# Scalsol/mega.pytorch

Hardware: AMD Instinct MI355X
Metric: frames/sec MEGA R-101 inference, 1000x600 VID clip (higher is better)
Workload: dtype bf16

## Files before the change

### mega/pytorch_amd/csrc/relation.hip

```cpp
#include <type_traits>

#include "launch.h"

namespace {

__device__ __forceinline__ void sincos_reduced(float a, float* sn, float* cs) {
  const float INV2PI = 0.15915494309189535f;
  const float TWO_PI_HI = 6.28318548202514648f;
  const float TWO_PI_LO = -1.7484555e-7f;
  const float n = rintf(a * INV2PI);
  float r = fmaf(-n, TWO_PI_HI, a);
  r = fmaf(-n, TWO_PI_LO, r);
  const float rev = r * INV2PI;
  *sn = __builtin_amdgcn_sinf(rev);
  *cs = __builtin_amdgcn_cosf(rev);
}

template <bool PRECISE>
__global__ __launch_bounds__(256) void pos_logits_kernel(const float4* __restrict__ rois_q,
                                                         const float4* __restrict__ rois_k,
                                                         const float* __restrict__ wgt, const float* __restrict__ bg,
                                                         const float* __restrict__ dim_mat, float* __restrict__ out,
                                                         int Nq, int Nk, int ldp) {
  __shared__ __attribute__((aligned(16))) float sw[64 * 16];
  __shared__ float sdim[8];
  for (int e = threadIdx.x; e < 1024; e += 256) sw[e] = wgt[e];
  if (threadIdx.x < 8) sdim[threadIdx.x] = dim_mat[threadIdx.x];
  __syncthreads();
  const int q = blockIdx.y;
  const int k = blockIdx.x * 256 + threadIdx.x;
  if (k >= Nk) return;
  const float4 bq = rois_q[q];
  const float4 bk = rois_k[k];
  const float wq = bq.z - bq.x + 1.f, hq = bq.w - bq.y + 1.f;
  const float cxq = 0.5f * (bq.x + bq.z), cyq = 0.5f * (bq.y + bq.w);
  const float wk = bk.z - bk.x + 1.f, hk = bk.w - bk.y + 1.f;
  const float cxk = 0.5f * (bk.x + bk.z), cyk = 0.5f * (bk.y + bk.w);
  float pm[4];
  pm[0] = logf(fabsf((cxq - cxk) / wq) + 1e-3f);
  pm[1] = logf(fabsf((cyq - cyk) / hq) + 1e-3f);
  pm[2] = logf(wq / wk);
  pm[3] = logf(hq / hk);
  float acc[16];
#pragma unroll
  for (int h = 0; h < 16; ++h) acc[h] = bg[h];
#pragma unroll
  for (int d = 0; d < 4; ++d) {
    const float pv = pm[d] * 100.0f;
#pragma unroll 2
    for (int i = 0; i < 8; ++i) {
      const float a = pv / sdim[i];
      float sn, cs;
      if (PRECISE) sincosf(a, &sn, &cs);
      else sincos_reduced(a, &sn, &cs);
      const float4* ws = reinterpret_cast<const float4*>(sw + (d * 16 + i) * 16);
      const float4* wc = reinterpret_cast<const float4*>(sw + (d * 16 + 8 + i) * 16);
#pragma unroll
      for (int h4 = 0; h4 < 4; ++h4) {
        const float4 a4 = ws[h4], c4 = wc[h4];
        acc[4 * h4 + 0] = fmaf(sn, a4.x, acc[4 * h4 + 0]);
        acc[4 * h4 + 1] = fmaf(sn, a4.y, acc[4 * h4 + 1]);
        acc[4 * h4 + 2] = fmaf(sn, a4.z, acc[4 * h4 + 2]);
        acc[4 * h4 + 3] = fmaf(sn, a4.w, acc[4 * h4 + 3]);
        acc[4 * h4 + 0] = fmaf(cs, c4.x, acc[4 * h4 + 0]);
        acc[4 * h4 + 1] = fmaf(cs, c4.y, acc[4 * h4 + 1]);
        acc[4 * h4 + 2] = fmaf(cs, c4.z, acc[4 * h4 + 2]);
        acc[4 * h4 + 3] = fmaf(cs, c4.w, acc[4 * h4 + 3]);
      }
    }
  }
#pragma unroll
  for (int h = 0; h < 16; ++h)
    out[((size_t)h * Nq + q) * ldp + k] = logf(fmaxf(acc[h], 0.f) + 1e-6f);
}

__device__ __forceinline__ float sin_shifted(float a, float shift_rev) {
  const float INV2PI = 0.15915494309189535f;
  const float TWO_PI_HI = 6.28318548202514648f;
  const float TWO_PI_LO = -1.7484555e-7f;
  const float n = rintf(a * INV2PI);
  float r = fmaf(-n, TWO_PI_HI, a);
  r = fmaf(-n, TWO_PI_LO, r);
  return __builtin_amdgcn_sinf(fmaf(r, INV2PI, shift_rev));
}

__device__ __forceinline__ float sin_rev(float x_rev) {
  return __builtin_amdgcn_sinf(__builtin_amdgcn_fractf(x_rev));
}

__device__ __forceinline__ float fast_log(float x) { return __builtin_amdgcn_logf(x) * 0.6931471805599453f; }
__device__ __forceinline__ float fast_div(float a, float b) { return a * __builtin_amdgcn_rcpf(b); }

typedef float f32x4_t __attribute__((ext_vector_type(4)));

__global__ __launch_bounds__(256) void pos_logits_mfma_kernel(const float4* __restrict__ rois_q,
                                                              const float4* __restrict__ rois_k,
                                                              const float* __restrict__ wgt,
                                                              const float* __restrict__ bg,
                                                              const float* __restrict__ dim_mat,
                                                              float* __restrict__ out, int Nq, int Nk, int ldp) {
  const int lane = threadIdx.x & 63, wave = threadIdx.x >> 6;
  const int row = lane & 15, g = lane >> 4;
  const int q = blockIdx.y;
  bf16x8_t bw[2];
#pragma unroll
  for (int s = 0; s < 2; ++s)
#pragma unroll
    for (int e = 0; e < 8; ++e) bw[s][e] = (__bf16)wgt[(32 * s + 8 * g + e) * 16 + row];
  float crev[8];
#pragma unroll
  for (int i = 0; i < 8; ++i) crev[i] = (100.0f * 0.15915494309189535f) / dim_mat[i];
  const float bias = bg[row];
  const float4 bq = rois_q[q];
  const float wq = bq.z - bq.x + 1.f, hq = bq.w - bq.y + 1.f;
  const float cxq = 0.5f * (bq.x + bq.z), cyq = 0.5f * (bq.y + bq.w);
  const float shift = (g & 1) ? 0.25f : 0.f;
#pragma unroll 1
  for (int t = 0; t < 4; ++t) {
    const int k0 = blockIdx.x * 256 + wave * 64 + t * 16;
    if (k0 >= Nk) break;
    const int k = min(k0 + row, Nk - 1);
    const float4 bk = rois_k[k];
    const float wk = bk.z - bk.x + 1.f, hk = bk.w - bk.y + 1.f;
    const float cxk = 0.5f * (bk.x + bk.z), cyk = 0.5f * (bk.y + bk.w);
    float pm[2];
    if (g >> 1) {
      pm[0] = fast_log(fabsf(fast_div(cyq - cyk, hq)) + 1e-3f);
      pm[1] = fast_log(fast_div(hq, hk));
    } else {
      pm[0] = fast_log(fabsf(fast_div(cxq - cxk, wq)) + 1e-3f);
      pm[1] = fast_log(fast_div(wq, wk));
    }
    f32x4_t acc = {bias, bias, bias, bias};
#pragma unroll
    for (int s = 0; s < 2; ++s) {
      bf16x8_t a;
#pragma unroll
      for (int i = 0; i < 8; ++i) a[i] = (__bf16)sin_rev(fmaf(pm[s], crev[i], shift));
      acc = __builtin_amdgcn_mfma_f32_16x16x32_bf16(a, bw[s], acc, 0, 0, 0);
    }
    float4 o;
    o.x = fast_log(fmaxf(acc[0], 0.f) + 1e-6f); o.y = fast_log(fmaxf(acc[1], 0.f) + 1e-6f);
    o.z = fast_log(fmaxf(acc[2], 0.f) + 1e-6f); o.w = fast_log(fmaxf(acc[3], 0.f) + 1e-6f);
    float* dst = out + ((size_t)row * Nq + q) * ldp + k0 + 4 * g;
    if (k0 + 4 * g + 3 < ldp) *reinterpret_cast<float4*>(dst) = o;
  }
}

template <typename HT> struct PosMma;
template <> struct PosMma<bf16_t> {
  typedef bf16x8_t vec;
  typedef __bf16 elem;
  __device__ static __forceinline__ f32x4_t run(const vec& a, const vec& b, const f32x4_t& c) { return __builtin_amdgcn_mfma_f32_16x16x32_bf16(a, b, c, 0, 0, 0); }
};
template <> struct PosMma<f16_t> {
  typedef f16x8_t vec;
  typedef _Float16 elem;
  __device__ static __forceinline__ f32x4_t run(const vec& a, const vec& b, const f32x4_t& c) { return __builtin_amdgcn_mfma_f32_16x16x32_f16(a, b, c, 0, 0, 0); }
};

template <typename HT>
__device__ __forceinline__ void pos_logits_tiled_body(const float4* __restrict__ rois_q,
                                                      const float4* __restrict__ rois_k,
                                                      const float* __restrict__ wgt, const float* __restrict__ bg,
                                                      const float* __restrict__ dim_mat, unsigned short* __restrict__ out_t,
                                                      int Nq, int Nk) {
  typedef typename PosMma<HT>::vec hvec;
  typedef typename PosMma<HT>::elem helem;
  __shared__ __attribute__((aligned(16))) unsigned short stage[16 * 2 * 8 * 32];
  const int lane = threadIdx.x & 63, wave = threadIdx.x >> 6;
  const int row = lane & 15, g = lane >> 4;
  const int q0 = blockIdx.y * 8, k00 = blockIdx.x * 64;
  hvec bw[2];
#pragma unroll
  for (int s = 0; s < 2; ++s)
#pragma unroll
    for (int e = 0; e < 8; ++e) bw[s][e] = (helem)wgt[(32 * s + 8 * g + e) * 16 + row];
  float crev[8];
#pragma unroll
  for (int i = 0; i < 8; ++i) crev[i] = (100.0f * 0.15915494309189535f) / dim_mat[i];
  const float bias = bg[row];
  const float shift = (g & 1) ? 0.25f : 0.f;
  float4 bqs[2], bks[4];
#pragma unroll
  for (int j = 0; j < 2; ++j) bqs[j] = rois_q[min(q0 + 2 * wave + j, Nq - 1)];
#pragma unroll
  for (int j = 0; j < 4; ++j) bks[j] = rois_k[min(k00 + j * 16 + row, Nk - 1)];
#pragma unroll
  for (int tile = 0; tile < 8; ++tile) {
    const int ql = 2 * wave + (tile >> 2);
    const int kb = (tile & 3) * 16;
    const float4 bq = bqs[tile >> 2];
    const float4 bk = bks[tile & 3];
    const float wq = bq.z - bq.x + 1.f, hq = bq.w - bq.y + 1.f;
    const float cxq = 0.5f * (bq.x + bq.z), cyq = 0.5f * (bq.y + bq.w);
    const float wk = bk.z - bk.x + 1.f, hk = bk.w - bk.y + 1.f;
    const float cxk = 0.5f * (bk.x + bk.z), cyk = 0.5f * (bk.y + bk.w);
    float pm[2];
    if (g >> 1) {
      pm[0] = fast_log(fabsf(fast_div(cyq - cyk, hq)) + 1e-3f);
      pm[1] = fast_log(fast_div(hq, hk));
    } else {
      pm[0] = fast_log(fabsf(fast_div(cxq - cxk, wq)) + 1e-3f);
      pm[1] = fast_log(fast_div(wq, wk));
    }
    f32x4_t acc = {bias, bias, bias, bias};
#pragma unroll
    for (int s = 0; s < 2; ++s) {
      hvec a;
#pragma unroll
      for (int i = 0; i < 8; ++i) a[i] = (helem)sin_rev(fmaf(pm[s], crev[i], shift));
      acc = PosMma<HT>::run(a, bw[s], acc);
    }
    const int kf = kb + 4 * g, ktl = kf >> 5, kk = kf & 31;
    uint2 pk;
    pk.x = Half16<HT>::pack2(fast_log(fmaxf(acc[0], 0.f) + 1e-6f), fast_log(fmaxf(acc[1], 0.f) + 1e-6f));
    pk.y = Half16<HT>::pack2(fast_log(fmaxf(acc[2], 0.f) + 1e-6f), fast_log(fmaxf(acc[3], 0.f) + 1e-6f));
    *reinterpret_cast<uint2*>(&stage[((row * 2 + ktl) * 8 + ql) * 32 + ((kk >> 2) & 1) * 16 + (kk >> 3) * 4]) = pk;
  }
  __syncthreads();
  const int ktiles = (Nk + 31) >> 5, kt0 = k00 >> 5;
  for (int idx = threadIdx.x; idx < 16 * 2 * 8 * 4; idx += 256) {
    const int chunk = idx & 3, ql = (idx >> 2) & 7, ktl = (idx >> 5) & 1, head = idx >> 6;
    if (q0 + ql < Nq && kt0 + ktl < ktiles)
      *reinterpret_cast<uint4*>(out_t + (((size_t)head * ktiles + kt0 + ktl) * Nq + q0 + ql) * 32 + chunk * 8) =
          *reinterpret_cast<const uint4*>(&stage[((head * 2 + ktl) * 8 + ql) * 32 + chunk * 8]);
  }
}

constexpr int POS_MAXB = 20;
struct PosBatch {
  struct { const float4* rq; const float4* rk; unsigned short* out; int Nq, Nk; } p[POS_MAXB];
};
template <typename HT>
__global__ __launch_bounds__(256) void pos_logits_tiled_batched_kernel(PosBatch b, const float* __restrict__ wgt,
                                                                       const float* __restrict__ bg,
                                                                       const float* __restrict__ dim_mat) {
  const auto& q = b.p[blockIdx.z];
  if ((int)blockIdx.x * 64 >= q.Nk || (int)blockIdx.y * 8 >= q.Nq) return;
  pos_logits_tiled_body<HT>(q.rq, q.rk, wgt, bg, dim_mat, q.out, q.Nq, q.Nk);
}

template <typename T> struct AttnCfg;
template <> struct AttnCfg<bf16_t> {
  static constexpr int KROW = 144;
  static constexpr int VROW = 72;
  static constexpr int NQF = 4;
  static constexpr int NPV = 2;
  static constexpr int NLD = 1;
};
template <> struct AttnCfg<f16_t> : AttnCfg<bf16_t> {};
template <> struct AttnCfg<float> {
  static constexpr int KROW = 272;
  static constexpr int VROW = 144;
  static constexpr int NQF = 8;
  static constexpr int NPV = 4;
  static constexpr int NLD = 2;
};

template <typename T> struct Mma32;
template <> struct Mma32<bf16_t> {
  __device__ static __forceinline__ void run(f32x16_t& acc, const uint4& a, const uint4& b) {
    acc = __builtin_amdgcn_mfma_f32_32x32x16_bf16(__builtin_bit_cast(bf16x8_t, a), __builtin_bit_cast(bf16x8_t, b), acc,
                                                  0, 0, 0);
  }
};
template <> struct Mma32<f16_t> {
  __device__ static __forceinline__ void run(f32x16_t& acc, const uint4& a, const uint4& b) {
    acc = __builtin_amdgcn_mfma_f32_32x32x16_f16(__builtin_bit_cast(f16x8_t, a), __builtin_bit_cast(f16x8_t, b), acc, 0, 0, 0);
  }
};
template <typename T> struct PairSum;
template <> struct PairSum<bf16_t> {
  __device__ static __forceinline__ float run(unsigned pk, float acc) {
    typedef __bf16 bf16x2_v __attribute__((ext_vector_type(2)));
    return __builtin_amdgcn_fdot2_f32_bf16(__builtin_bit_cast(bf16x2_v, pk), __builtin_bit_cast(bf16x2_v, 0x3f803f80u), acc, false);
  }
};
template <> struct PairSum<f16_t> {
  __device__ static __forceinline__ float run(unsigned pk, float acc) {
    return __builtin_amdgcn_fdot2(__builtin_bit_cast(f16x2_t, pk), __builtin_bit_cast(f16x2_t, 0x3c003c00u), acc, false);
  }
};
template <> struct PairSum<float> {
  __device__ static __forceinline__ float run(unsigned, float acc) { return acc; }
};
template <> struct Mma32<float> {
  __device__ static __forceinline__ void run(f32x16_t& acc, const uint4& a, const uint4& b) {
    acc = __builtin_amdgcn_mfma_f32_32x32x2f32(__uint_as_float(a.x), __uint_as_float(b.x), acc, 0, 0, 0);
    acc = __builtin_amdgcn_mfma_f32_32x32x2f32(__uint_as_float(a.y), __uint_as_float(b.y), acc, 0, 0, 0);
    acc = __builtin_amdgcn_mfma_f32_32x32x2f32(__uint_as_float(a.z), __uint_as_float(b.z), acc, 0, 0, 0);
    acc = __builtin_amdgcn_mfma_f32_32x32x2f32(__uint_as_float(a.w), __uint_as_float(b.w), acc, 0, 0, 0);
  }
};


struct AttnParams {
  const void* Q;
  const void* K;
  const void* Vt;
  const void* K2;
  const void* Vt2;
  const float* pos;
  const unsigned short* pos_t;
  const void* resid;
  const float* bias_v;
  void* out;
  float* part_o;
  float* part_ml;
  int ldq, ldk, ldv, ldv2, ldp, ldr, ldo;
  int Nq, Nk, N1, G;
  float scale;
  int nsplit, tiles_per_split;
  int io_f32;
};

template <typename T, bool POS_TILED, bool SEG>
__device__ __forceinline__ void attn_body(const AttnParams& p, const int split) {
  using C = AttnCfg<T>;
  constexpr int VE = 16 / (int)sizeof(T);
  constexpr int KV_PER_ROW = 64 * (int)sizeof(T) / 16;
  constexpr int VV_PER_ROW = 32 * (int)sizeof(T) / 16;
  constexpr int NLD = C::NLD;
  __shared__ __attribute__((aligned(16))) unsigned char Ks[2][32 * C::KROW];
  __shared__ __attribute__((aligned(16))) unsigned char Vs[2][64 * C::VROW];
  __shared__ __attribute__((aligned(16))) float sRow[4][32];

  const int tid = threadIdx.x, lane = tid & 63, wave = tid >> 6;
  const int h2 = lane >> 5, l31 = lane & 31;
  const int head = blockIdx.y;
  const int qw0 = blockIdx.x * 128 + wave * 32;
  const bool live = !POS_TILED || __builtin_amdgcn_readfirstlane(qw0) < p.Nq;
  const T* __restrict__ Qp = (const T*)p.Q;
  const int N1 = SEG ? p.N1 : p.Nk;
  const __amdgpu_buffer_rsrc_t rs_k = __builtin_amdgcn_make_buffer_rsrc(
      const_cast<void*>(p.K), 0, (int)((unsigned)N1 * (unsigned)p.ldk * (unsigned)sizeof(T)), 0x00020000);
  const __amdgpu_buffer_rsrc_t rs_v = __builtin_amdgcn_make_buffer_rsrc(
      const_cast<void*>(p.Vt), 0, (int)((unsigned)(p.G * 64) * (unsigned)p.ldv * (unsigned)sizeof(T)), 0x00020000);
  const __amdgpu_buffer_rsrc_t rs_k2 = __builtin_amdgcn_make_buffer_rsrc(
      const_cast<void*>(p.K2), 0, (int)((unsigned)(p.Nk - N1) * (unsigned)p.ldk * (unsigned)sizeof(T)), 0x00020000);
  const __amdgpu_buffer_rsrc_t rs_v2 = __builtin_amdgcn_make_buffer_rsrc(
      const_cast<void*>(p.Vt2), 0, (int)((unsigned)(p.G * 64) * (unsigned)p.ldv2 * (unsigned)sizeof(T)), 0x00020000);

  const int q_ld = min(qw0 + l31, p.Nq - 1);
  uint4 qf[C::NQF];
  {
    const unsigned char* qrow = (const unsigned char*)(Qp + (size_t)q_ld * p.ldq + head * 64);
#pragma unroll
    for (int v = 0; v < C::NQF; ++v) qf[v] = *reinterpret_cast<const uint4*>(qrow + v * 32 + h2 * 16);
  }

  auto load_tiles = [&](int k0, uint4 (&kreg)[NLD], uint4 (&vreg)[NLD]) {
    const bool in1 = !SEG || k0 + 32 <= N1, in2 = SEG && k0 >= N1;
#pragma unroll
    for (int i = 0; i < NLD; ++i) {
      const int idx = tid + 256 * i;
      {
        const int row = idx / KV_PER_ROW, vec = idx - row * KV_PER_ROW;
        const int key = k0 + row;
        const unsigned col = (unsigned)(head * 64 + vec * VE);
        const unsigned off1 = ((unsigned)key * (unsigned)p.ldk + col) * (unsigned)sizeof(T);
        const unsigned off2 = ((unsigned)(key - N1) * (unsigned)p.ldk + col) * (unsigned)sizeof(T);
        u32x4_t v;
        if (in1) {
          v = __builtin_amdgcn_raw_buffer_load_b128(rs_k, key < N1 ? off1 : 0xFFFFFFFFu, 0, 0);
        } else if (!SEG) {
          v = u32x4_t{0, 0, 0, 0};
        } else if (in2) {
          v = __builtin_amdgcn_raw_buffer_load_b128(rs_k2, key < p.Nk ? off2 : 0xFFFFFFFFu, 0, 0);
        } else {
          const u32x4_t a = __builtin_amdgcn_raw_buffer_load_b128(rs_k, key < N1 ? off1 : 0xFFFFFFFFu, 0, 0);
          const u32x4_t b = __builtin_amdgcn_raw_buffer_load_b128(rs_k2, key >= N1 && key < p.Nk ? off2 : 0xFFFFFFFFu, 0, 0);
          v = a | b;
        }
        kreg[i] = make_uint4(v.x, v.y, v.z, v.w);
      }
      {
        const int row = idx / VV_PER_ROW, vec = idx - row * VV_PER_ROW;
        const int key = k0 + vec * VE;
        const unsigned off1 = ((unsigned)(head * 64 + row) * (unsigned)p.ldv + (unsigned)key) * (unsigned)sizeof(T);
        const unsigned off2 = ((unsigned)(head * 64 + row) * (unsigned)p.ldv2 + (unsigned)(key - N1)) * (unsigned)sizeof(T);
        u32x4_t r;
        if (in1) {
          r = __builtin_amdgcn_raw_buffer_load_b128(rs_v, key < N1 ? off1 : 0xFFFFFFFFu, 0, 0);
        } else if (!SEG) {
          r = u32x4_t{0, 0, 0, 0};
        } else if (in2) {
          r = __builtin_amdgcn_raw_buffer_load_b128(rs_v2, key < p.Nk ? off2 : 0xFFFFFFFFu, 0, 0);
        } else {
          const u32x4_t a = __builtin_amdgcn_raw_buffer_load_b128(rs_v, key + VE <= N1 ? off1 : 0xFFFFFFFFu, 0, 0);
          const u32x4_t b = __builtin_amdgcn_raw_buffer_load_b128(rs_v2, key >= N1 && key < p.Nk ? off2 : 0xFFFFFFFFu, 0, 0);
          r = a | b;
          if (key < N1 && key + VE > N1) {
            T e[VE];
#pragma unroll
            for (int t = 0; t < VE; ++t) {
              const int kk = key + t;
              const T* src = kk < N1 ? (const T*)p.Vt + (size_t)(head * 64 + row) * p.ldv + kk
                                     : (const T*)p.Vt2 + (size_t)(head * 64 + row) * p.ldv2 + (kk - N1);
              e[t] = kk < p.Nk ? *src : (T)0;
            }
            r = *reinterpret_cast<const u32x4_t*>(e);
          }
        }
        uint4 v = make_uint4(r.x, r.y, r.z, r.w);
        if (k0 + 32 > p.Nk) {
          T* e = reinterpret_cast<T*>(&v);
#pragma unroll
          for (int t = 0; t < VE; ++t) e[t] = (key + t < p.Nk) ? e[t] : (T)0;
        }
        vreg[i] = v;
      }
    }
  };
  auto store_tiles = [&](int buf, const uint4 (&kreg)[NLD], const uint4 (&vreg)[NLD]) {
#pragma unroll
    for (int i = 0; i < NLD; ++i) {
      const int idx = tid + 256 * i;
      {
        const int row = idx / KV_PER_ROW, vec = idx - row * KV_PER_ROW;
        *reinterpret_cast<uint4*>(&Ks[buf][row * C::KROW + vec * 16]) = kreg[i];
      }
      {
        const int row = idx / VV_PER_ROW, vec = idx - row * VV_PER_ROW;
        unsigned char* dst = &Vs[buf][row * C::VROW + vec * 16];
        if (sizeof(T) == 2) {
          *reinterpret_cast<uint2*>(dst) = make_uint2(vreg[i].x, vreg[i].y);
          *reinterpret_cast<uint2*>(dst + 8) = make_uint2(vreg[i].z, vreg[i].w);
        } else {
          *reinterpret_cast<uint4*>(dst) = vreg[i];
        }
      }
    }
  };

  f32x16_t o0, o1;
#pragma unroll
  for (int r = 0; r < 16; ++r) { o0[r] = 0.f; o1[r] = 0.f; }
  float m_run = -INFINITY, l_run = 0.f;
  const float* pos_row = p.pos ? p.pos + ((size_t)head * p.Nq + q_ld) * p.ldp : nullptr;
  const int ktiles = (p.Nk + 31) >> 5;
  auto load_pos = [&](int kt, uint4 (&pr)[2]) {
    if (POS_TILED) {
      const int kc = min(kt, ktiles - 1);
      const uint4* src = reinterpret_cast<const uint4*>(p.pos_t + (((size_t)head * ktiles + kc) * p.Nq + q_ld) * 32 + h2 * 16);
      pr[0] = src[0];
      pr[1] = src[1];
    }
  };

  auto compute = [&](int cur, int k0, const uint4 (&pr)[2]) {
    f32x16_t st;
#pragma unroll
    for (int r = 0; r < 16; ++r) st[r] = 0.f;
    {
      const unsigned char* kb = &Ks[cur][l31 * C::KROW + h2 * 16];
#pragma unroll
      for (int v = 0; v < C::NQF; ++v) {
        const uint4 kf = *reinterpret_cast<const uint4*>(kb + v * 32);
        Mma32<T>::run(st, kf, qf[v]);
      }
    }
    float s[16];
#pragma unroll
    for (int rq = 0; rq < 4; ++rq) {
      float pe[4] = {0.f, 0.f, 0.f, 0.f};
      if (POS_TILED) {
        const unsigned short* pb = reinterpret_cast<const unsigned short*>(&pr[0]);
#pragma unroll
        for (int e = 0; e < 4; ++e) pe[e] = Half16<typename std::conditional<sizeof(T) == 2, T, bf16_t>::type>::one(pb[4 * rq + e]);
      } else if (pos_row) {
        const float4 pw = *reinterpret_cast<const float4*>(pos_row + k0 + 8 * rq + 4 * h2);
        pe[0] = pw.x; pe[1] = pw.y; pe[2] = pw.z; pe[3] = pw.w;
      }
#pragma unroll
      for (int e = 0; e < 4; ++e) s[4 * rq + e] = st[4 * rq + e] * p.scale + pe[e];
    }
    if (k0 + 32 > p.Nk) {
#pragma unroll
      for (int r = 0; r < 16; ++r) {
        const int key = k0 + 8 * (r >> 2) + 4 * h2 + (r & 3);
        s[r] = key < p.Nk ? s[r] : -INFINITY;
      }
    }
    float mt = s[0];
#pragma unroll
    for (int r = 1; r < 16; ++r) mt = fmaxf(mt, s[r]);
    mt = fmaxf(mt, __shfl_xor(mt, 32));
    const float m_new = fmaxf(m_run, mt);
    auto ex = [](float v) { return sizeof(T) == 2 ? __expf(v) : expf(v); };
    const float alpha = ex(m_run - m_new);
    float psum = 0.f;
    unsigned pk[8];
    if (sizeof(T) == 2) {
      const float kL2E = 1.44269504088896340736f, mneg = -m_new * kL2E;
#pragma unroll
      for (int r = 0; r < 16; ++r) s[r] = __builtin_amdgcn_exp2f(fmaf(s[r], kL2E, mneg));
    } else {
#pragma unroll
      for (int r = 0; r < 16; ++r) s[r] = ex(s[r] - m_new);
    }
    if (sizeof(T) == 2) {
#pragma unroll
      for (int d = 0; d < 8; ++d) {
        pk[d] = Half16<typename std::conditional<sizeof(T) == 2, T, bf16_t>::type>::pack2(s[2 * d], s[2 * d + 1]);
        psum = PairSum<T>::run(pk[d], psum);
      }
    } else {
#pragma unroll
      for (int r = 0; r < 16; ++r) psum += s[r];
    }
    l_run = l_run * alpha + psum;
    m_run = m_new;

    if (__builtin_amdgcn_ballot_w64(alpha != 1.f) != 0) {
      if (h2 == 0) sRow[wave][l31] = alpha;
      __builtin_amdgcn_wave_barrier();
#pragma unroll
      for (int rq = 0; rq < 4; ++rq) {
        const float4 a4 = *reinterpret_cast<const float4*>(&sRow[wave][8 * rq + 4 * h2]);
        o0[4 * rq + 0] *= a4.x; o0[4 * rq + 1] *= a4.y; o0[4 * rq + 2] *= a4.z; o0[4 * rq + 3] *= a4.w;
        o1[4 * rq + 0] *= a4.x; o1[4 * rq + 1] *= a4.y; o1[4 * rq + 2] *= a4.z; o1[4 * rq + 3] *= a4.w;
      }
      __builtin_amdgcn_wave_barrier();
    }

    const unsigned char* vb0 = &Vs[cur][l31 * C::VROW];
    const unsigned char* vb1 = &Vs[cur][(32 + l31) * C::VROW];
#pragma unroll
    for (int u = 0; u < C::NPV; ++u) {
      uint4 pa, v0, v1;
      if (sizeof(T) == 2) {
        pa.x = pk[4 * u + 0];
        pa.y = pk[4 * u + 1];
        pa.z = pk[4 * u + 2];
        pa.w = pk[4 * u + 3];
        const int off = (16 * u + 4 * h2) * 2;
        const uint2 a0 = *reinterpret_cast<const uint2*>(vb0 + off);
        const uint2 a1 = *reinterpret_cast<const uint2*>(vb0 + off + 16);
        const uint2 b0 = *reinterpret_cast<const uint2*>(vb1 + off);
        const uint2 b1 = *reinterpret_cast<const uint2*>(vb1 + off + 16);
        v0 = make_uint4(a0.x, a0.y, a1.x, a1.y);
        v1 = make_uint4(b0.x, b0.y, b1.x, b1.y);
      } else {
        pa.x = __float_as_uint(s[4 * u + 0]);
        pa.y = __float_as_uint(s[4 * u + 1]);
        pa.z = __float_as_uint(s[4 * u + 2]);
        pa.w = __float_as_uint(s[4 * u + 3]);
        const int off = (8 * u + 4 * h2) * 4;
        v0 = *reinterpret_cast<const uint4*>(vb0 + off);
        v1 = *reinterpret_cast<const uint4*>(vb1 + off);
      }
      Mma32<T>::run(o0, pa, v0);
      Mma32<T>::run(o1, pa, v1);
    }
  };

  const int ntiles = (p.Nk + 31) / 32;
  const int t0 = split * p.tiles_per_split;
  const int n = min(ntiles, t0 + p.tiles_per_split) - t0;
  uint4 ka[NLD], va[NLD], kb2[NLD], vb2[NLD];
  uint4 pA[2] = {}, pB[2] = {};
  load_tiles(t0 * 32, ka, va);
  load_pos(t0, pA);
  store_tiles(0, ka, va);
  load_tiles((t0 + 1) * 32, ka, va);
  load_pos(t0 + 1, pB);
  __syncthreads();
  for (int i = 0; i + 1 < n; i += 2) {
    load_tiles((t0 + i + 2) * 32, kb2, vb2);
    if (live) {
      compute(0, (t0 + i) * 32, pA);
      load_pos(t0 + i + 2, pA);
    }
    store_tiles(1, ka, va);
    __syncthreads();
    load_tiles((t0 + i + 3) * 32, ka, va);
    if (live) {
      compute(1, (t0 + i + 1) * 32, pB);
      load_pos(t0 + i + 3, pB);
    }
    store_tiles(0, kb2, vb2);
    __syncthreads();
  }
  if (!live) return;
  if (n & 1) compute(0, (t0 + n - 1) * 32, pA);

  const float l_tot = l_run + __shfl_xor(l_run, 32);
  if (p.nsplit > 1) {
    if (h2 == 0 && qw0 + l31 < p.Nq) {
      float* ml = p.part_ml + (size_t)split * 2 * p.G * p.Nq;
      ml[(size_t)head * p.Nq + qw0 + l31] = m_run;
      ml[(size_t)(p.G + head) * p.Nq + qw0 + l31] = l_tot;
    }
    float* po = p.part_o + (size_t)split * p.Nq * p.G * 64;
#pragma unroll
    for (int jj = 0; jj < 2; ++jj) {
      const int col = head * 64 + jj * 32 + l31;
#pragma unroll
      for (int r = 0; r < 16; ++r) {
        const int q = qw0 + (r & 3) + 8 * (r >> 2) + 4 * h2;
        if (q < p.Nq) po[(size_t)q * p.G * 64 + col] = (jj == 0 ? o0[r] : o1[r]);
      }
    }
    return;
  }
  if (h2 == 0) sRow[wave][l31] = 1.f / l_tot;
  __builtin_amdgcn_wave_barrier();
  const T* __restrict__ resid = (const T*)p.resid;
  T* __restrict__ out = (T*)p.out;
#pragma unroll
  for (int jj = 0; jj < 2; ++jj) {
    const int col = head * 64 + jj * 32 + l31;
    const float bv = p.bias_v ? p.bias_v[col] : 0.f;
#pragma unroll
    for (int r = 0; r < 16; ++r) {
      const int ql = (r & 3) + 8 * (r >> 2) + 4 * h2;
      const int q = qw0 + ql;
      if (q < p.Nq) {
        float v = (jj == 0 ? o0[r] : o1[r]) * sRow[wave][ql] + bv;
        if (p.io_f32) {
          if (resid) v += reinterpret_cast<const float*>(p.resid)[(size_t)q * p.ldr + col];
          reinterpret_cast<float*>(p.out)[(size_t)q * p.ldo + col] = v;
        } else {
          if (resid) v += Elem<T>::ld(resid + (size_t)q * p.ldr + col);
          Elem<T>::st(out + (size_t)q * p.ldo + col, v);
        }
      }
    }
  }
}

constexpr int ATTN_MAXB = 20;
constexpr int ATTN_MAXZ = 256;
struct AttnBatch {
  int n, nz;
  unsigned char zprob[ATTN_MAXZ], zsplit[ATTN_MAXZ];
  AttnParams p[ATTN_MAXB];
};
static_assert(sizeof(AttnBatch) <= 4096, "AttnBatch travels as the kernel argument");

template <typename T, bool POS_TILED, bool SEG>
__global__ __launch_bounds__(256, (POS_TILED && SEG) ? 3 : 2) void attn_batched_kernel(AttnBatch b) {
  const int z = blockIdx.z;
  const AttnParams& p = b.p[b.zprob[z]];
  if ((int)blockIdx.x * 128 >= p.Nq) return;
  attn_body<T, POS_TILED, SEG>(p, (int)b.zsplit[z]);
}

template <typename T>
__device__ __forceinline__ void attn_combine_body(const AttnParams& p) {
  const int D = p.G * 64;
  const size_t total = (size_t)p.Nq * D;
  for (size_t idx = (size_t)blockIdx.x * blockDim.x + threadIdx.x; idx < total; idx += (size_t)gridDim.x * blockDim.x) {
    const int q = (int)(idx / D), c = (int)(idx - (size_t)q * D), head = c >> 6;
    float M = -INFINITY;
    for (int s = 0; s < p.nsplit; ++s)
      M = fmaxf(M, p.part_ml[((size_t)s * 2 * p.G + head) * p.Nq + q]);
    float num = 0.f, den = 0.f;
    for (int s = 0; s < p.nsplit; ++s) {
      const float* ml = p.part_ml + (size_t)s * 2 * p.G * p.Nq;
      const float w = expf(ml[(size_t)head * p.Nq + q] - M);
      den += w * ml[(size_t)(p.G + head) * p.Nq + q];
      num += w * p.part_o[((size_t)s * p.Nq + q) * D + c];
    }
    float v = num / den + (p.bias_v ? p.bias_v[c] : 0.f);
    if (p.io_f32) {
      if (p.resid) v += reinterpret_cast<const float*>(p.resid)[(size_t)q * p.ldr + c];
      reinterpret_cast<float*>(p.out)[(size_t)q * p.ldo + c] = v;
    } else {
      if (p.resid) v += Elem<T>::ld((const T*)p.resid + (size_t)q * p.ldr + c);
      Elem<T>::st((T*)p.out + (size_t)q * p.ldo + c, v);
    }
  }
}

template <typename T>
__global__ __launch_bounds__(256) void attn_combine_batched_kernel(AttnBatch b) {
  const AttnParams& p = b.p[blockIdx.y];
  if (p.nsplit > 1) attn_combine_body<T>(p);
}

inline size_t align_up(size_t x, size_t a) { return (x + a - 1) / a * a; }

}

extern "C" int mega_position_logits(const float* rois_q, const float* rois_k, const float* wg_t, const float* bg,
                                    const float* dim_mat, float* out, int Nq, int Nk, int ldp, int precise,
                                    void* stream) {
  mega_clear_error();
  if (Nq == 0 || Nk == 0) return MEGA_OK;
  if (!rois_q || !rois_k || !wg_t || !bg || !dim_mat || !out || Nq < 0 || Nk < 0 || ldp < Nk) return MEGA_ERR_ARG;
  dim3 grid(cdiv(Nk, 256), Nq);
  if (precise)
    hipLaunchKernelGGL((pos_logits_kernel<true>), grid, dim3(256), 0, (hipStream_t)stream, (const float4*)rois_q,
                       (const float4*)rois_k, wg_t, bg, dim_mat, out, Nq, Nk, ldp);
  else if (ldp % 4 == 0 && (reinterpret_cast<size_t>(out) & 15) == 0)
    hipLaunchKernelGGL(pos_logits_mfma_kernel, grid, dim3(256), 0, (hipStream_t)stream, (const float4*)rois_q,
                       (const float4*)rois_k, wg_t, bg, dim_mat, out, Nq, Nk, ldp);
  else
    hipLaunchKernelGGL((pos_logits_kernel<false>), grid, dim3(256), 0, (hipStream_t)stream, (const float4*)rois_q,
                       (const float4*)rois_k, wg_t, bg, dim_mat, out, Nq, Nk, ldp);
  return mega_check_launch();
}

struct MegaPosDescC { const float* rois_q; const float* rois_k; void* out_bf16; int Nq, Nk; };

static int pos_tiled_launch(const MegaPosDescC* d, int n, const float* wg_t, const float* bg, const float* dim_mat,
                            int dtype, void* stream) {
  if (!d || n < 0 || n > POS_MAXB || !wg_t || !bg || !dim_mat) return MEGA_ERR_ARG;
  PosBatch b;
  int max_q = 0, max_k = 0;
  for (int i = 0; i < n; ++i) {
    if (!d[i].rois_q || !d[i].rois_k || !d[i].out_bf16 || d[i].Nq <= 0 || d[i].Nk <= 0 ||
        (reinterpret_cast<size_t>(d[i].out_bf16) & 15))
      return MEGA_ERR_ARG;
    b.p[i].rq = (const float4*)d[i].rois_q; b.p[i].rk = (const float4*)d[i].rois_k; b.p[i].out = (unsigned short*)d[i].out_bf16;
    b.p[i].Nq = d[i].Nq; b.p[i].Nk = d[i].Nk;
    max_q = d[i].Nq > max_q ? d[i].Nq : max_q;
    max_k = d[i].Nk > max_k ? d[i].Nk : max_k;
  }
  dim3 grid(cdiv(max_k, 64), cdiv(max_q, 8), n);
  return dispatch_half(dtype, [&](auto tag) {
    hipLaunchKernelGGL(pos_logits_tiled_batched_kernel<decltype(tag)>, grid, dim3(256), 0, (hipStream_t)stream, b, wg_t, bg,
                       dim_mat);
    return mega_check_launch();
  });
}

extern "C" int mega_position_logits_tiled_dt(const float* rois_q, const float* rois_k, const float* wg_t, const float* bg,
                                             const float* dim_mat, void* out16, int Nq, int Nk, int dtype, void* stream) {
  mega_clear_error();
  if (dtype != MEGA_BF16 && dtype != MEGA_F16) return MEGA_ERR_ARG;
  if (Nq == 0 || Nk == 0) return MEGA_OK;
  const MegaPosDescC d = {rois_q, rois_k, out16, Nq, Nk};
  return pos_tiled_launch(&d, 1, wg_t, bg, dim_mat, dtype, stream);
}

extern "C" int mega_position_logits_tiled_batched_dt(const void* descs, int n, const float* wg_t, const float* bg,
                                                     const float* dim_mat, int dtype, void* stream) {
  mega_clear_error();
  if (dtype != MEGA_BF16 && dtype != MEGA_F16) return MEGA_ERR_ARG;
  if (n == 0) return MEGA_OK;
  return pos_tiled_launch((const MegaPosDescC*)descs, n, wg_t, bg, dim_mat, dtype, stream);
}

constexpr int kAttnTargetBlocks = 48;

extern "C" int mega_relation_attention_splits(int Nq, int Nk, int groups) {
  if (Nq <= 0 || Nk <= 0 || groups <= 0) return 1;
  const int blocks = cdiv(Nq, 128) * groups;
  const int ntiles = cdiv(Nk, 32);
  int s = cdiv(kAttnTargetBlocks, blocks);
  if (s > ntiles / 4) s = ntiles / 4;
  if (s > 16) s = 16;
  return s < 1 ? 1 : s;
}

extern "C" size_t mega_relation_attention_workspace_bytes(int Nq, int Nk, int groups) {
  const int s = mega_relation_attention_splits(Nq, Nk, groups);
  if (s <= 1) return 0;
  return align_up((size_t)s * Nq * groups * 64 * sizeof(float), 256) +
         align_up((size_t)s * 2 * groups * Nq * sizeof(float), 256);
}

static int attn_fill(AttnParams& p, const void* q, int ldq, const void* k, int ldk, const void* vt, int ldv,
                     const float* pos, int ldp, const void* pos_tiled, const void* resid, int ldr, const float* bias_v,
                     void* out, int ldo, int Nq, int Nk, int groups, float scale, int dtype, void* ws, size_t ws_bytes,
                     int io_f32 = 0, int nk1 = 0, const void* k2 = nullptr, const void* vt2 = nullptr, int ldv2 = 0) {
  if (!q || !k || !vt || !out || Nq <= 0 || Nk <= 0 || groups <= 0) return MEGA_ERR_ARG;
  if (nk1 < 0 || nk1 > Nk) return MEGA_ERR_ARG;
  if (nk1 == 0 || nk1 == Nk) { nk1 = Nk; k2 = k; vt2 = vt; ldv2 = ldv; }
  else if (!k2 || !vt2 || ldv2 < Nk - nk1) return MEGA_ERR_ARG;
  p.N1 = nk1; p.K2 = k2; p.Vt2 = vt2; p.ldv2 = ldv2;
  p.io_f32 = (io_f32 != 0 && dtype != MEGA_F32) ? 1 : 0;
  const int ve = dtype != MEGA_F32 ? 8 : 4;
  if (ldq % ve || ldk % ve || ldv % ve || (pos && (ldp % 32 || ldp < Nk))) return MEGA_ERR_ARG;
  if (ldv < (nk1 == Nk ? ((Nk + ve - 1) / ve) * ve : nk1)) return MEGA_ERR_ARG;
  if (pos_tiled && (pos || dtype == MEGA_F32 || (reinterpret_cast<size_t>(pos_tiled) & 15))) return MEGA_ERR_ARG;
  p.pos_t = (const unsigned short*)pos_tiled;
  p.Q = q; p.ldq = ldq; p.K = k; p.ldk = ldk; p.Vt = vt; p.ldv = ldv; p.pos = pos; p.ldp = ldp;
  p.resid = resid; p.ldr = ldr; p.bias_v = bias_v; p.out = out; p.ldo = ldo; p.Nq = Nq; p.Nk = Nk; p.G = groups;
  p.scale = scale;
  const int want = mega_relation_attention_splits(Nq, Nk, groups);
  int nsplit = want;
  if (nsplit > 1 && (!ws || ws_bytes < mega_relation_attention_workspace_bytes(Nq, Nk, groups))) nsplit = 1;
  const int ntiles = cdiv(Nk, 32);
  p.tiles_per_split = cdiv(ntiles, nsplit);
  nsplit = cdiv(ntiles, p.tiles_per_split);
  p.nsplit = nsplit;
  p.part_o = (float*)ws;
  p.part_ml = nsplit > 1 ? (float*)((unsigned char*)ws + align_up((size_t)want * Nq * groups * 64 * sizeof(float), 256))
                         : nullptr;
  return MEGA_OK;
}

struct MegaAttnDescC {
  const void* q; const void* k; const void* vt; const float* pos; const void* pos_tiled; const void* resid;
  const float* bias_v; void* out; void* ws; size_t ws_bytes;
  int ldq, ldk, ldv, ldp, ldr, ldo, Nq, Nk;
  int io_f32, nk1;
  const void* k2; const void* vt2; int ldv2, reserved;
};

static int attn_launch(const MegaAttnDescC* d, int n, int groups, float scale, int dtype, void* stream) {
  if (!d || n < 0 || n > ATTN_MAXB) return MEGA_ERR_ARG;
  AttnBatch b;
  b.n = n;
  int nz = 0, max_q = 0, any_split = 0, any_seg = 0;
  size_t max_total = 0;
  const bool tiled = d[0].pos_tiled != nullptr;
  for (int i = 0; i < n; ++i) {
    if ((d[i].pos_tiled != nullptr) != tiled) return MEGA_ERR_ARG;
    const int rc = attn_fill(b.p[i], d[i].q, d[i].ldq, d[i].k, d[i].ldk, d[i].vt, d[i].ldv, d[i].pos, d[i].ldp,
                             d[i].pos_tiled, d[i].resid, d[i].ldr, d[i].bias_v, d[i].out, d[i].ldo, d[i].Nq, d[i].Nk,
                             groups, scale, dtype, d[i].ws, d[i].ws_bytes, d[i].io_f32, d[i].nk1, d[i].k2, d[i].vt2,
                             d[i].ldv2);
    if (rc != MEGA_OK) return rc;
    if (nz + b.p[i].nsplit > ATTN_MAXZ) return MEGA_ERR_ARG;
    for (int s2 = 0; s2 < b.p[i].nsplit; ++s2) { b.zprob[nz] = (unsigned char)i; b.zsplit[nz] = (unsigned char)s2; ++nz; }
    max_q = d[i].Nq > max_q ? d[i].Nq : max_q;
    any_split |= b.p[i].nsplit > 1;
    any_seg |= b.p[i].N1 != b.p[i].Nk;
    const size_t total = (size_t)d[i].Nq * groups * 64;
    max_total = total > max_total ? total : max_total;
  }
  b.nz = nz;
  hipStream_t st = (hipStream_t)stream;
  dim3 grid(cdiv(max_q, 128), groups, nz);
  return dispatch_elem(dtype, [&](auto tag) {
    using T = decltype(tag);
    auto kernel = any_seg ? attn_batched_kernel<T, false, true> : attn_batched_kernel<T, false, false>;
    if constexpr (!std::is_same<T, float>::value)
      if (tiled) kernel = any_seg ? attn_batched_kernel<T, true, true> : attn_batched_kernel<T, true, false>;
    hipLaunchKernelGGL(kernel, grid, dim3(256), 0, st, b);
    if (any_split)
      hipLaunchKernelGGL(attn_combine_batched_kernel<T>, dim3(grid1d(max_total, 4096), n), dim3(256), 0, st, b);
    return mega_check_launch();
  });
}

extern "C" int mega_relation_attention_batched(const void* descs, int n, int groups, float scale, int dtype,
                                               void* stream) {
  mega_clear_error();
  if (n == 0) return MEGA_OK;
  return attn_launch((const MegaAttnDescC*)descs, n, groups, scale, dtype, stream);
}

static int relation_attention_impl(const void* q, int ldq, const void* k, int ldk, const void* vt, int ldv,
                                   const float* pos, int ldp, const void* pos_tiled, const void* resid, int ldr,
                                   const float* bias_v, void* out, int ldo, int Nq, int Nk, int groups, float scale,
                                   int dtype, void* ws, size_t ws_bytes, void* stream) {
  mega_clear_error();
  if (Nq == 0) return MEGA_OK;
  MegaAttnDescC d = {};
  d.q = q; d.k = k; d.vt = vt; d.pos = pos; d.pos_tiled = pos_tiled; d.resid = resid; d.bias_v = bias_v; d.out = out;
  d.ws = ws; d.ws_bytes = ws_bytes;
  d.ldq = ldq; d.ldk = ldk; d.ldv = ldv; d.ldp = ldp; d.ldr = ldr; d.ldo = ldo; d.Nq = Nq; d.Nk = Nk;
  return attn_launch(&d, 1, groups, scale, dtype, stream);
}

extern "C" int mega_relation_attention(const void* q, int ldq, const void* k, int ldk, const void* vt, int ldv,
                                       const float* pos, int ldp, const void* resid, int ldr, const float* bias_v,
                                       void* out, int ldo, int Nq, int Nk, int groups, float scale, int dtype,
                                       void* ws, size_t ws_bytes, void* stream) {
  return relation_attention_impl(q, ldq, k, ldk, vt, ldv, pos, ldp, nullptr, resid, ldr, bias_v, out, ldo, Nq, Nk,
                                 groups, scale, dtype, ws, ws_bytes, stream);
}

extern "C" int mega_relation_attention_tiled_pos_dt(const void* q, int ldq, const void* k, int ldk, const void* vt,
                                                    int ldv, const void* pos_tiled16, const void* resid, int ldr,
                                                    const float* bias_v, void* out, int ldo, int Nq, int Nk, int groups,
                                                    float scale, int dtype, void* ws, size_t ws_bytes, void* stream) {
  if (dtype != MEGA_BF16 && dtype != MEGA_F16) return MEGA_ERR_ARG;
  return relation_attention_impl(q, ldq, k, ldk, vt, ldv, nullptr, 0, pos_tiled16, resid, ldr, bias_v, out, ldo, Nq,
                                 Nk, groups, scale, dtype, ws, ws_bytes, stream);
}
```

Baseline: 944.0.

## Prefetch tiled position logits via buffer-to-LDS DMA with counted waits

For the tiled positional-bias path, position logit tiles now go straight into per-wave LDS with buffer_load_lds, four tiles deep, instead of register loads two tiles ahead. Reads use counted vmcnt waits and inline-asm ds_reads for K and V fragments. Barriers become raw s_barrier. Seam handling is moved to store time with a single load at load time, tail zeroing is deferred to the store, and non-live waves get a separate loop. The aim is to hide global latency on the positional stream and cut VGPR and instruction overhead. In exchange it adds LDS use (32KB per block, asserted to fit three blocks per CU) and fragile hand-counted waitcnt logic.

```diff
diff --git a/mega/pytorch_amd/csrc/relation.hip b/mega/pytorch_amd/csrc/relation.hip
--- a/mega/pytorch_amd/csrc/relation.hip
+++ b/mega/pytorch_amd/csrc/relation.hip
@@ -241,6 +241,8 @@
   pos_logits_tiled_body<HT>(q.rq, q.rk, wgt, bg, dim_mat, q.out, q.Nq, q.Nk);
 }
 
+typedef __attribute__((address_space(3))) void* lds_ptr_t;
+typedef unsigned int u32x2_t __attribute__((ext_vector_type(2)));
 template <typename T> struct AttnCfg;
 template <> struct AttnCfg<bf16_t> {
   static constexpr int KROW = 144;
@@ -325,6 +327,9 @@
   __shared__ __attribute__((aligned(16))) unsigned char Ks[2][32 * C::KROW];
   __shared__ __attribute__((aligned(16))) unsigned char Vs[2][64 * C::VROW];
   __shared__ __attribute__((aligned(16))) float sRow[4][32];
+  constexpr int PD = 4;
+  __shared__ __attribute__((aligned(16))) unsigned char Ps[POS_TILED ? 4 * PD * 2048 : 16];
+  static_assert(sizeof(Ks) + sizeof(Vs) + sizeof(sRow) + sizeof(Ps) <= 160 * 1024 / 3 || !POS_TILED, "three blocks per CU");
 
   const int tid = threadIdx.x, lane = tid & 63, wave = tid >> 6;
   const int h2 = lane >> 5, l31 = lane & 31;
@@ -350,6 +355,8 @@
     for (int v = 0; v < C::NQF; ++v) qf[v] = *reinterpret_cast<const uint4*>(qrow + v * 32 + h2 * 16);
   }
 
+  constexpr bool ZERO_AT_STORE = POS_TILED;
+  constexpr bool ONE_LOAD = SEG && POS_TILED;
   auto load_tiles = [&](int k0, uint4 (&kreg)[NLD], uint4 (&vreg)[NLD]) {
     const bool in1 = !SEG || k0 + 32 <= N1, in2 = SEG && k0 >= N1;
 #pragma unroll
@@ -362,7 +369,10 @@
         const unsigned off1 = ((unsigned)key * (unsigned)p.ldk + col) * (unsigned)sizeof(T);
         const unsigned off2 = ((unsigned)(key - N1) * (unsigned)p.ldk + col) * (unsigned)sizeof(T);
         u32x4_t v;
-        if (in1) {
+        if (ONE_LOAD) {
+          v = __builtin_amdgcn_raw_buffer_load_b128(in2 ? rs_k2 : rs_k, in2 ? (key < p.Nk ? off2 : 0xFFFFFFFFu)
+                                                                            : (key < N1 ? off1 : 0xFFFFFFFFu), 0, 0);
+        } else if (in1) {
           v = __builtin_amdgcn_raw_buffer_load_b128(rs_k, key < N1 ? off1 : 0xFFFFFFFFu, 0, 0);
         } else if (!SEG) {
           v = u32x4_t{0, 0, 0, 0};
@@ -381,7 +391,10 @@
         const unsigned off1 = ((unsigned)(head * 64 + row) * (unsigned)p.ldv + (unsigned)key) * (unsigned)sizeof(T);
         const unsigned off2 = ((unsigned)(head * 64 + row) * (unsigned)p.ldv2 + (unsigned)(key - N1)) * (unsigned)sizeof(T);
         u32x4_t r;
-        if (in1) {
+        if (ONE_LOAD) {
+          r = __builtin_amdgcn_raw_buffer_load_b128(in2 ? rs_v2 : rs_v, in2 ? (key < p.Nk ? off2 : 0xFFFFFFFFu)
+                                                                            : (key + VE <= N1 ? off1 : 0xFFFFFFFFu), 0, 0);
+        } else if (in1) {
           r = __builtin_amdgcn_raw_buffer_load_b128(rs_v, key < N1 ? off1 : 0xFFFFFFFFu, 0, 0);
         } else if (!SEG) {
           r = u32x4_t{0, 0, 0, 0};
@@ -404,7 +417,7 @@
           }
         }
         uint4 v = make_uint4(r.x, r.y, r.z, r.w);
-        if (k0 + 32 > p.Nk) {
+        if (!ZERO_AT_STORE && k0 + 32 > p.Nk) {
           T* e = reinterpret_cast<T*>(&v);
 #pragma unroll
           for (int t = 0; t < VE; ++t) e[t] = (key + t < p.Nk) ? e[t] : (T)0;
@@ -413,20 +426,52 @@
       }
     }
   };
-  auto store_tiles = [&](int buf, const uint4 (&kreg)[NLD], const uint4 (&vreg)[NLD]) {
+  auto store_tiles = [&](int buf, int k0, const uint4 (&kreg)[NLD], const uint4 (&vreg)[NLD]) {
 #pragma unroll
     for (int i = 0; i < NLD; ++i) {
       const int idx = tid + 256 * i;
+      const bool seam = ONE_LOAD && k0 < N1 && k0 + 32 > N1;
       {
         const int row = idx / KV_PER_ROW, vec = idx - row * KV_PER_ROW;
-        *reinterpret_cast<uint4*>(&Ks[buf][row * C::KROW + vec * 16]) = kreg[i];
+        uint4 kv = kreg[i];
+        if (seam) {
+          const int key = k0 + row;
+          const unsigned off2 = ((unsigned)(key - N1) * (unsigned)p.ldk + (unsigned)(head * 64 + vec * VE)) * (unsigned)sizeof(T);
+          const u32x4_t b = __builtin_amdgcn_raw_buffer_load_b128(rs_k2, key >= N1 && key < p.Nk ? off2 : 0xFFFFFFFFu, 0, 0);
+          kv.x |= b.x; kv.y |= b.y; kv.z |= b.z; kv.w |= b.w;
+        }
+        *reinterpret_cast<uint4*>(&Ks[buf][row * C::KROW + vec * 16]) = kv;
       }
       {
         const int row = idx / VV_PER_ROW, vec = idx - row * VV_PER_ROW;
         unsigned char* dst = &Vs[buf][row * C::VROW + vec * 16];
         if (sizeof(T) == 2) {
-          *reinterpret_cast<uint2*>(dst) = make_uint2(vreg[i].x, vreg[i].y);
-          *reinterpret_cast<uint2*>(dst + 8) = make_uint2(vreg[i].z, vreg[i].w);
+          uint4 v = vreg[i];
+          if (seam) {
+            const int key = k0 + vec * VE;
+            const unsigned off2 = ((unsigned)(head * 64 + row) * (unsigned)p.ldv2 + (unsigned)(key - N1)) * (unsigned)sizeof(T);
+            const u32x4_t b = __builtin_amdgcn_raw_buffer_load_b128(rs_v2, key >= N1 && key < p.Nk ? off2 : 0xFFFFFFFFu, 0, 0);
+            v.x |= b.x; v.y |= b.y; v.z |= b.z; v.w |= b.w;
+            if (key < N1 && key + VE > N1) {
+              T e[VE];
+#pragma unroll
+              for (int t = 0; t < VE; ++t) {
+                const int kk = key + t;
+                const T* src = kk < N1 ? (const T*)p.Vt + (size_t)(head * 64 + row) * p.ldv + kk
+                                       : (const T*)p.Vt2 + (size_t)(head * 64 + row) * p.ldv2 + (kk - N1);
+                e[t] = kk < p.Nk ? *src : (T)0;
+              }
+              v = *reinterpret_cast<const uint4*>(e);
+            }
+          }
+          if (ZERO_AT_STORE && k0 + 32 > p.Nk) {
+            const int key = k0 + vec * VE;
+            T* e = reinterpret_cast<T*>(&v);
+#pragma unroll
+            for (int t = 0; t < VE; ++t) e[t] = (key + t < p.Nk) ? e[t] : (T)0;
+          }
+          *reinterpret_cast<uint2*>(dst) = make_uint2(v.x, v.y);
+          *reinterpret_cast<uint2*>(dst + 8) = make_uint2(v.z, v.w);
         } else {
           *reinterpret_cast<uint4*>(dst) = vreg[i];
         }
@@ -440,12 +485,33 @@
   float m_run = -INFINITY, l_run = 0.f;
   const float* pos_row = p.pos ? p.pos + ((size_t)head * p.Nq + q_ld) * p.ldp : nullptr;
   const int ktiles = (p.Nk + 31) >> 5;
-  auto load_pos = [&](int kt, uint4 (&pr)[2]) {
+  const __amdgpu_buffer_rsrc_t rs_p = __builtin_amdgcn_make_buffer_rsrc(
+      const_cast<unsigned short*>(POS_TILED ? p.pos_t + (size_t)head * ktiles * p.Nq * 32 : nullptr), 0,
+      (int)((unsigned)ktiles * (unsigned)p.Nq * 64u), 0x00020000);
+  unsigned pq_off[2];
+#pragma unroll
+  for (int j = 0; j < 2; ++j) pq_off[j] = (unsigned)min(qw0 + 16 * j + (lane >> 2), p.Nq - 1) * 64u + (unsigned)(lane & 3) * 16u;
+  unsigned char* const ps_wave = &Ps[POS_TILED ? wave * PD * 2048 : 0];
+  auto dma_pos = [&](int kt) {
     if (POS_TILED) {
-      const int kc = min(kt, ktiles - 1);
-      const uint4* src = reinterpret_cast<const uint4*>(p.pos_t + (((size_t)head * ktiles + kc) * p.Nq + q_ld) * 32 + h2 * 16);
-      pr[0] = src[0];
-      pr[1] = src[1];
+      const unsigned plane = (unsigned)min(kt, ktiles - 1) * (unsigned)p.Nq * 64u;
+      unsigned char* dst = ps_wave + (kt & (PD - 1)) * 2048;
+#pragma unroll
+      for (int j = 0; j < 2; ++j)
+        __builtin_amdgcn_raw_ptr_buffer_load_lds(rs_p, (lds_ptr_t)(dst + j * 1024), 16, pq_off[j], plane, 0, 0);
+    }
+  };
+  const unsigned ps_rd = (unsigned)(size_t)(lds_ptr_t)ps_wave + (unsigned)(l31 * 64 + h2 * 32);
+  auto read_pos = [&](int kt, uint4 (&pr)[2], auto vm_after) {
+    if (POS_TILED) {
+      constexpr int VM_AFTER = decltype(vm_after)::value;
+      u32x4_t a, b;
+      asm volatile("s_waitcnt vmcnt(%3)\n\tds_read_b128 %0, %2\n\tds_read_b128 %1, %2 offset:16\n\ts_waitcnt lgkmcnt(0)"
+                   : "=&v"(a), "=&v"(b)
+                   : "v"(ps_rd + (unsigned)((kt & (PD - 1)) * 2048)), "n"(VM_AFTER)
+                   : "memory");
+      pr[0] = make_uint4(a.x, a.y, a.z, a.w);
+      pr[1] = make_uint4(b.x, b.y, b.z, b.w);
     }
   };
 
@@ -453,7 +519,19 @@
     f32x16_t st;
 #pragma unroll
     for (int r = 0; r < 16; ++r) st[r] = 0.f;
-    {
+    if (POS_TILED) {
+      u32x4_t kf[4];
+      const unsigned ka = (unsigned)(size_t)(lds_ptr_t)&Ks[cur][l31 * C::KROW + h2 * 16];
+#define MEGA_ATTN_RD128(dst, addr, imm) asm volatile("ds_read_b128 %0, %1 offset:%2" : "=v"(dst) : "v"(addr), "n"(imm) : "memory")
+      MEGA_ATTN_RD128(kf[0], ka, 0);
+      MEGA_ATTN_RD128(kf[1], ka, 32);
+      MEGA_ATTN_RD128(kf[2], ka, 64);
+      MEGA_ATTN_RD128(kf[3], ka, 96);
+      asm volatile("s_waitcnt lgkmcnt(0)" : "+v"(kf[0]), "+v"(kf[1]), "+v"(kf[2]), "+v"(kf[3])::"memory");
+#pragma unroll
+      for (int v = 0; v < 4; ++v) Mma32<T>::run(st, make_uint4(kf[v].x, kf[v].y, kf[v].z, kf[v].w), qf[v]);
+#undef MEGA_ATTN_RD128
+    } else {
       const unsigned char* kb = &Ks[cur][l31 * C::KROW + h2 * 16];
 #pragma unroll
       for (int v = 0; v < C::NQF; ++v) {
@@ -527,10 +605,33 @@
 
     const unsigned char* vb0 = &Vs[cur][l31 * C::VROW];
     const unsigned char* vb1 = &Vs[cur][(32 + l31) * C::VROW];
+    u32x2_t vf[8];
+    if (POS_TILED) {
+      const unsigned va = (unsigned)(size_t)(lds_ptr_t)&Vs[cur][l31 * C::VROW + h2 * 8];
+#define MEGA_ATTN_RD64(dst, addr, imm) asm volatile("ds_read_b64 %0, %1 offset:%2" : "=v"(dst) : "v"(addr), "n"(imm) : "memory")
+      MEGA_ATTN_RD64(vf[0], va, 0);
+      MEGA_ATTN_RD64(vf[1], va, 16);
+      MEGA_ATTN_RD64(vf[2], va, 32 * C::VROW);
+      MEGA_ATTN_RD64(vf[3], va, 32 * C::VROW + 16);
+      MEGA_ATTN_RD64(vf[4], va, 32);
+      MEGA_ATTN_RD64(vf[5], va, 48);
+      MEGA_ATTN_RD64(vf[6], va, 32 * C::VROW + 32);
+      MEGA_ATTN_RD64(vf[7], va, 32 * C::VROW + 48);
+#undef MEGA_ATTN_RD64
+      asm volatile("s_waitcnt lgkmcnt(0)"
+                   : "+v"(vf[0]), "+v"(vf[1]), "+v"(vf[2]), "+v"(vf[3]), "+v"(vf[4]), "+v"(vf[5]), "+v"(vf[6]), "+v"(vf[7])::"memory");
+    }
 #pragma unroll
     for (int u = 0; u < C::NPV; ++u) {
       uint4 pa, v0, v1;
-      if (sizeof(T) == 2) {
+      if (POS_TILED) {
+        pa.x = pk[4 * u + 0];
+        pa.y = pk[4 * u + 1];
+        pa.z = pk[4 * u + 2];
+        pa.w = pk[4 * u + 3];
+        v0 = make_uint4(vf[4 * u + 0].x, vf[4 * u + 0].y, vf[4 * u + 1].x, vf[4 * u + 1].y);
+        v1 = make_uint4(vf[4 * u + 2].x, vf[4 * u + 2].y, vf[4 * u + 3].x, vf[4 * u + 3].y);
+      } else if (sizeof(T) == 2) {
         pa.x = pk[4 * u + 0];
         pa.y = pk[4 * u + 1];
         pa.z = pk[4 * u + 2];
@@ -556,35 +657,70 @@
     }
   };
 
+  auto tile_barrier = [&]() {
+    if (POS_TILED) {
+      asm volatile("s_waitcnt lgkmcnt(0)" ::: "memory");
+      __builtin_amdgcn_s_barrier();
+      asm volatile("" ::: "memory");
+    } else {
+      __syncthreads();
+    }
+  };
+
   const int ntiles = (p.Nk + 31) / 32;
   const int t0 = split * p.tiles_per_split;
   const int n = min(ntiles, t0 + p.tiles_per_split) - t0;
   uint4 ka[NLD], va[NLD], kb2[NLD], vb2[NLD];
-  uint4 pA[2] = {}, pB[2] = {};
+  uint4 pr[2] = {};
+  constexpr int kPosVmAfter = 2 * (PD - 1) + 2 * NLD * PD;
+  static_assert(!POS_TILED || (NLD == 1 && kPosVmAfter == 14), "the counted wait of read_pos");
+  if (POS_TILED && !live) {
+    load_tiles(t0 * 32, ka, va);
+    store_tiles(0, t0 * 32, ka, va);
+    load_tiles((t0 + 1) * 32, ka, va);
+    tile_barrier();
+    for (int i = 0; i + 1 < n; i += 2) {
+      load_tiles((t0 + i + 2) * 32, kb2, vb2);
+      store_tiles(1, (t0 + i + 1) * 32, ka, va);
+      tile_barrier();
+      load_tiles((t0 + i + 3) * 32, ka, va);
+      store_tiles(0, (t0 + i + 2) * 32, kb2, vb2);
+      tile_barrier();
+    }
+    return;
+  }
   load_tiles(t0 * 32, ka, va);
-  load_pos(t0, pA);
-  store_tiles(0, ka, va);
+  if (live)
+    for (int d = 0; d < PD; ++d) dma_pos(t0 + d);
+  store_tiles(0, t0 * 32, ka, va);
   load_tiles((t0 + 1) * 32, ka, va);
-  load_pos(t0 + 1, pB);
-  __syncthreads();
+  if (POS_TILED && live) asm volatile("s_waitcnt vmcnt(0)" ::: "memory");
+  tile_barrier();
   for (int i = 0; i + 1 < n; i += 2) {
     load_tiles((t0 + i + 2) * 32, kb2, vb2);
     if (live) {
-      compute(0, (t0 + i) * 32, pA);
-      load_pos(t0 + i + 2, pA);
-    }
-    store_tiles(1, ka, va);
-    __syncthreads();
+      read_pos(t0 + i, pr, std::integral_constant<int, kPosVmAfter>());
+      compute(0, (t0 + i) * 32, pr);
+      dma_pos(t0 + i + PD);
+    }
+    store_tiles(1, (t0 + i + 1) * 32, ka, va);
+    tile_barrier();
     load_tiles((t0 + i + 3) * 32, ka, va);
     if (live) {
-      compute(1, (t0 + i + 1) * 32, pB);
-      load_pos(t0 + i + 3, pB);
-    }
-    store_tiles(0, kb2, vb2);
-    __syncthreads();
+      read_pos(t0 + i + 1, pr, std::integral_constant<int, kPosVmAfter>());
+      compute(1, (t0 + i + 1) * 32, pr);
+      dma_pos(t0 + i + 1 + PD);
+    }
+    store_tiles(0, (t0 + i + 2) * 32, kb2, vb2);
+    tile_barrier();
   }
   if (!live) return;
-  if (n & 1) compute(0, (t0 + n - 1) * 32, pA);
+  if (n & 1) {
+    read_pos(t0 + n - 1, pr, std::integral_constant<int, 0>());
+    compute(0, (t0 + n - 1) * 32, pr);
+  } else if (POS_TILED) {
+    asm volatile("s_waitcnt vmcnt(0)" ::: "memory");
+  }
 
   const float l_tot = l_run + __shfl_xor(l_run, 32);
   if (p.nsplit > 1) {
@@ -778,6 +914,7 @@
   if (ldq % ve || ldk % ve || ldv % ve || (pos && (ldp % 32 || ldp < Nk))) return MEGA_ERR_ARG;
   if (ldv < (nk1 == Nk ? ((Nk + ve - 1) / ve) * ve : nk1)) return MEGA_ERR_ARG;
   if (pos_tiled && (pos || dtype == MEGA_F32 || (reinterpret_cast<size_t>(pos_tiled) & 15))) return MEGA_ERR_ARG;
+  if (pos_tiled && (unsigned long long)cdiv(Nk, 32) * (unsigned long long)Nq * 64ull > 0x7FFFFFFFull) return MEGA_ERR_ARG;
   p.pos_t = (const unsigned short*)pos_tiled;
   p.Q = q; p.ldq = ldq; p.K = k; p.ldk = ldk; p.Vt = vt; p.ldv = ldv; p.pos = pos; p.ldp = ldp;
   p.resid = resid; p.ldr = ldr; p.bias_v = bias_v; p.out = out; p.ldo = ldo; p.Nq = Nq; p.Nk = Nk; p.G = groups;
```

After: 944.9, median of 2. Within noise of the previous version (+0.1%).
